# panuelosj/polystokes

Hardware: NVIDIA B200
Metric: stokes_steps_per_sec_256cubed (higher is better)
Workload: dtype f64

## Files before the change

### polystokes_b200/csrc/ps_api.cu

```cuda
#include "ps_solver.hpp"
#include <map>
#include <array>
#include <fstream>
#include <limits>
#include <thread>
#include <mutex>
#include <condition_variable>
#include <functional>
#include <memory>
#include <chrono>

using namespace ps;

struct MultiGroup;
struct ps_solver { Solver* S; void* tm[2] = {nullptr, nullptr}; Scratch scratch; MultiGroup* multi = nullptr; };

struct MultiGroup {
    struct Worker {
        std::thread th; std::mutex m; std::condition_variable cv;
        std::function<int()> task; bool has = false, quit = false, done = true; int rc = 0; std::string err;
        std::vector<void*> graveyard;
        const char* volatile where = "idle";
    };
    std::vector<ps_solver*> kids;
// ... 213 lines not shown
    if (name == "Mr") { out = blockdiag_csr(R ? S.RG.Mr.to_host(S.st, R * NN) : std::vector<double>(), R); return true; }
    if (name == "BInv") { out = blockdiag_csr(R ? S.RG.Binv.to_host(S.st, R * NN) : std::vector<double>(), R); return true; }
    if (name == "B") {
        std::vector<double> b(R * NN);
        if (R) { auto m = S.RG.Mr.to_host(S.st, R * NN); auto v = S.RG.Visc.to_host(S.st, R * NN); for (size_t i = 0; i < b.size(); ++i) b[i] = S.g.invDt * m[i] + 2. * v[i]; }
        out = blockdiag_csr(b, R); return true;
    }
    return false;
}
void mask_region_blocks(const Solver& S, const std::string& name, HostCsr& m) {
    if (!S.part.multi() || !(name == "Mr" || name == "B" || name == "BInv")) return;
    const size_t NN = (size_t)RDOF * RDOF;
    for (size_t i = 0; i < m.val.size(); ++i) { const int r = (int)(i / NN); if (r < S.RG.regLo || r >= S.RG.regHi) m.val[i] = 0.; }
}

bool get_vector(Solver& S, const std::string& n, std::vector<double>& out) {
    const Counts& C = S.C; const int R = S.RG.count; const size_t NN = (size_t)RDOF * RDOF;
    if (n == "activeRHS") out = S.rhsU.to_host(S.st, (size_t)C.nActiveVs);
    else if (n == "oldActiveVs") out = S.oldVs.to_host(S.st, (size_t)C.nActiveVs);
    else if (n == "reducedRHS") out = R ? S.RG.rhsR.to_host(S.st, (size_t)R * RDOF) : std::vector<double>();
    else if (n == "pressureRHS") out = S.rhsPT.to_host(S.st, (size_t)C.nPressures);
    else if (n == "stressRHS") { auto v = S.rhsPT.to_host(S.st, (size_t)C.nSystemSize); out.assign(v.begin() + C.nPressures, v.end()); }
    else if (n == "b") out = S.b.to_host(S.st, (size_t)C.nSystemSize);
    else if (n == "solution") out = S.x.to_host(S.st, (size_t)C.nSystemSize);
    else if (n == "velSolution") out = S.velSol.to_host(S.st, (size_t)(C.nActiveVs + C.nReducedVs));
    else if (n == "com") out = R ? S.RG.com.to_host(S.st, (size_t)3 * R) : std::vector<double>();
    else if (n == "bestFit") out = R ? S.RG.bestFit.to_host(S.st, (size_t)R * RDOF) : std::vector<double>();
    else if (n == "MrDense") out = R ? S.RG.Mr.to_host(S.st, R * NN) : std::vector<double>();
    else if (n == "ViscDense") out = R ? S.RG.Visc.to_host(S.st, R * NN) : std::vector<double>();
    else if (n == "BinvDense") out = R ? S.RG.Binv.to_host(S.st, R * NN) : std::vector<double>();
    else if (n == "guess") { if (S.guess.n < (size_t)C.nSystemSize) out.assign((size_t)C.nSystemSize, 0.); else out = S.guess.to_host(S.st, (size_t)C.nSystemSize); }
    else if (n == "diagA") { if (S.part.multi()) return false; S.computeDiagonal(); out = S.diagA.to_host(S.st, (size_t)C.nSystemSize); }
    else return false;
    if (S.part.multi()) {
        if (n == "b" || n == "solution") { for (size_t i = 0; i < out.size(); ++i) if (!S.ownSys.has((int64_t)i)) out[i] = 0.; }
        else if (n == "velSolution") {
            for (size_t i = 0; i < out.size(); ++i) {
                const bool mine = (int64_t)i < C.nActiveVs ? S.ownK.has((int64_t)i) : ((int64_t)(i - C.nActiveVs) / RDOF >= S.RG.regLo && (int64_t)(i - C.nActiveVs) / RDOF < S.RG.regHi);
                if (!mine) out[i] = 0.;
            }
        } else if (n == "reducedRHS" || n == "bestFit" || n == "MrDense" || n == "ViscDense" || n == "BinvDense") {
            const size_t per = (n == "reducedRHS" || n == "bestFit") ? (size_t)RDOF : NN;
            for (size_t i = 0; i < out.size(); ++i) { const int r = (int)(i / per); if (r < S.RG.regLo || r >= S.RG.regHi) out[i] = 0.; }
        }
    }
    return true;
}
// ... 199 lines not shown
    if (n == "nCenter") return C.nCenter;
    if (n == "nFaceX") return C.nFace[0]; if (n == "nFaceY") return C.nFace[1]; if (n == "nFaceZ") return C.nFace[2];
    if (n == "nEdgeYZ") return C.nEdge[0]; if (n == "nEdgeXZ") return C.nEdge[1]; if (n == "nEdgeXY") return C.nEdge[2];
    if (n == "nActiveVs") return C.nActiveVs; if (n == "nReducedVs") return C.nReducedVs;
    if (n == "nPressures") return C.nPressures; if (n == "nStresses") return C.nStresses;
    if (n == "nTotalDOFs") return C.nTotalDOFs; if (n == "nSystemSize") return C.nSystemSize;
    if (n == "regionCount") return S.RG.count; if (n == "iterations") return S.solveIterations;
    if (n == "peerTransport") return S.peer.on ? 1 : 0;
    if (n == "slabLocal") return S.part.local ? 1 : 0;
    if (n == "directHalo") return S.fusedHalo ? 1 : 0;
    if (n == "result") return S.result; if (n == "usedBiCGStab") return S.usedBiCGStab;
    if (n == "nRowsExt") return C.nRowsExt; if (n == "fixLoops") return S.fixLoops;
    if (n == "maxRegionRows") return S.RG.maxRegionRows; if (n == "maxRegionAxisRows") return S.RG.maxRegionAxisRows;
    if (n == "maxRegionCells") return S.RG.maxRegionCells; if (n == "minRegionCells") return S.RG.minRegionCells;
    if (n == "regionPath") return region_path(S.make_op_args(), S.RG);
    return INT64_MIN;
}
double ps_get_real(ps_handle h, const char* name) {
    if (!h || !name) return NAN;
    const std::string n(name);
    if (n == "solveError") return h->S->solveError;
    if (n == "xmag") return h->S->solveXmag;
    return NAN;
}

int64_t ps_get_index_field(ps_handle h, int kind, int slot, int32_t* out) {
    if (!h || slot < 0 || slot >= N_SLOTS || kind < 0 || kind > 2) return -1;
    if (h->multi) { g_lastError = "ps_get_index_field: per-voxel views of a ps_create_multi handle live on several GPUs; use a single-GPU handle"; return -1; }
    Solver& S = *h->S;
    const size_t n = (size_t)S.g.n[slot];
// ... 48 lines not shown
        dx.alloc(n); dy.alloc(n);
        copy_h2d(dx.p, x, n * sizeof(double), S.st);
        dy.zero(S.st, n);
        S.applyOperator(dx.p, dy.p, nullptr);
        copy_d2h(y, dy.p, n * sizeof(double), S.st);
        return (int)PS_SUCCESS;
    });
}

double ps_kernel_bytes(ps_handle h, const char* name) {
    if (!h || !name) return 0;
    const Solver& S = *h->S; const Counts& C = S.C; const std::string nm(name);
    const double nE = (double)(C.nEdge[0] + C.nEdge[1] + C.nEdge[2]);
    const double n = (double)C.nSystemSize;
    const double nRed = (double)S.RG.nRows;
    const double pass1Sweep = 32.0 * C.nRowsExt + 1.0 * C.nActiveVs  + 8.0 * n  + 8.0 * C.nRowsExt ;
    const double pass2 = 32.0 * C.nCenter + 20.0 * nE  + 8.0 * C.nRowsExt  + 8.0 * (C.nCenter + nE)
                       + 8.0 * n  + 8.0 * n ;
    const double pass2Dots = pass2 + 8.0 * n ;
    const double csrPass1 = 12.0 * 8.0 * C.nRowsExt + 8.0 * n + 8.0 * C.nActiveVs + 8.0 * C.nRowsExt;
    const double csrPass2 = 12.0 * (6.0 * C.nPressures + 2.0 * 3 * C.nCenter + 4.0 * nE) + 8.0 * C.nRowsExt + 8.0 * C.nStresses + 8.0 * C.nStresses + 8.0 * n;
    if (nm == "csr_pass1") return csrPass1;
    if (nm == "csr_pass2") return csrPass2;
    if (nm == "csr_apply") return csrPass1 + csrPass2 + nRed * 24.0 + (double)S.RG.count * (RDOF * RDOF + 2 * RDOF + 30) * 8.0;
    const double reduced = nRed * (8.0 + 4.0) + nRed * (4.0 + 8.0) + (double)S.RG.count * (RDOF * RDOF + 2 * RDOF + 30) * 8.0;
    const double pass1 = pass1Sweep + reduced;
    if (nm == "pass1") return pass1;
    if (nm == "pass1_sweep") return pass1Sweep;
    if (nm == "pass2") return pass2;
    if (nm == "pass2_dots") return pass2Dots;
    if (nm == "reduced") return reduced;
    if (nm == "apply") return pass1 + pass2;
// ... 112 lines not shown
```

### polystokes_b200/csrc/ps_assemble.cu

```cuda
#include "ps_solver.hpp"

namespace ps {

PS_D float local_viscosity_a(const Geom& g, const float* visc, int slot, const I3& idx) {
    int o[3] = {1, 1, 1};
    if (slot >= SL_FACE && slot < SL_EDGE) o[slot - SL_FACE] = 0;
    else if (slot >= SL_EDGE) { for (int a = 0; a < 3; ++a) if (a != slot - SL_EDGE) o[a] = 0; }
    const int b0 = o[0] ? idx.x : idx.x - 1, b1 = o[1] ? idx.y : idx.y - 1, b2 = o[2] ? idx.z : idx.z - 1;
    const float t0 = o[0] ? 0.f : 0.5f, t1 = o[1] ? 0.f : 0.5f, t2 = o[2] ? 0.f : 0.5f;
    float cz[2];
    for (int dz = 0; dz < 2; ++dz) {
        float cy[2];
        for (int dy = 0; dy < 2; ++dy) {
            const float a = float_at(g, visc, SL_CENTER, I3{b0, b1 + dy, b2 + dz});
            const float b = float_at(g, visc, SL_CENTER, I3{b0 + 1, b1 + dy, b2 + dz});
            cy[dy] = fadd_rn(a, fmul_rn(t0, fsub_rn(b, a)));
        }
        cz[dz] = fadd_rn(cy[0], fmul_rn(t1, fsub_rn(cy[1], cy[0])));
    }
    return fadd_rn(cz[0], fmul_rn(t2, fsub_rn(cz[1], cz[0])));
}

PS_D double clampd(double v, double lo, double hi) { return fmin(fmax(v, lo), hi); }

// ... 178 lines not shown
                }
            }
            const int64_t erow = eRowOff + ei;
            ecode[erow] = (uint32_t)word;
            for (int k = 0; k < 4; ++k) ecol[(int64_t)k * nERows + erow] = cidx[k];
            rhsPT[nP + tOff + ei] = rhs;
            const double volumeWeight = clampd((double)fwe * 0.125, MINWEIGHT, 1.0) * ((double)lw * 0.125);
            const double localViscosity = (double)local_viscosity_a(g, visc, SL_EDGE + e, ed);
            const double invLocalViscosity = clampd(1. / localViscosity, 0., 1e10);
            uInv[tOff + ei] = mul_rn(mul_rn(2., invLocalViscosity), volumeWeight);
            uDiag[tOff + ei] = mul_rn(mul_rn(0.5, localViscosity), clampd(1. / volumeWeight, 0., 1.e2));
        });
    }
}

}
```

### polystokes_b200/csrc/ps_pcg.cu

```cuda
#include "ps_solver.hpp"
#include "ps_peer.hpp"

namespace ps {

PS_D double k_row(const OpArgs& A, int64_t r, const double* __restrict__ x) {
    const uint64_t word = A.kcode[r];
    const int32_t c0w = A.kcol[r];
    const int64_t cOff = A.nP + (int64_t)((uint32_t)c0w >> 30) * A.nC;
    int64_t col[8];
    col[0] = c0w & OP_COL_MASK; col[1] = A.kcol[A.nRowsExt + r]; col[2] = cOff + col[0]; col[3] = cOff + col[1];
    for (int k = 0; k < 4; ++k) col[4 + k] = A.kcol[(int64_t)(2 + k) * A.nRowsExt + r];
    double s = 0.;
    for (int k = 0; k < 8; ++k) { const int code = op_code(word, k); if (code) s += ((double)code * A.valScale) * x[col[k]]; }
    return s;
}
PS_D void kt_cell_rows(const OpArgs& A, int64_t ci, const double* __restrict__ w, double* out) {
    const uint64_t word = A.ccode[ci];
    double v[6], wv[6];
    for (int k = 0; k < 6; ++k) { const int code = op_code(word, k); v[k] = (double)code * A.valScale; wv[k] = code ? w[A.ccol[(int64_t)k * A.nC + ci]] : 0.; }
    double s = 0.;
    for (int k = 0; k < 6; ++k) s += v[k] * wv[k];
    out[0] = s;
    for (int a = 0; a < 3; ++a) { double t = 0.; t += (-v[2 * a]) * wv[2 * a]; t += (-v[2 * a + 1]) * wv[2 * a + 1]; out[1 + a] = t; }
}
PS_D double kt_edge_row(const OpArgs& A, int64_t e, const double* __restrict__ w) {
    const uint64_t word = A.ecode[e];
    double s = 0.;
    for (int k = 0; k < 4; ++k) { const int code = op_code(word, k); if (code) s += ((double)code * A.valScale) * w[A.ecol[(int64_t)k * A.nE + e]]; }
    return s;
}

PS_D void moments_to_t(const double* M, double* t) {
    for (int n = 0; n < RDOF; ++n) t[n] = 0.;
    const double* A = M; const double* B = M + 10; const double* Cz = M + 20;
    t[0] = A[0]; t[3] = A[1]; t[4] = A[2]; t[5] = A[3]; for (int k = 0; k < 6; ++k) t[6 + k] = A[4 + k];
    t[1] = B[0]; t[12] = B[1]; t[13] = B[2]; t[14] = B[3]; for (int k = 0; k < 6; ++k) t[15 + k] = B[4 + k];
    t[2] += Cz[0]; t[3] += -Cz[3]; t[6] += -2. * Cz[6]; t[7] += -Cz[8]; t[8] += -0.5 * Cz[9];
    t[13] += -Cz[3]; t[16] += -Cz[6]; t[18] += -2. * Cz[8]; t[19] += -0.5 * Cz[9];
    t[21] += Cz[1]; t[22] += Cz[2]; t[23] += Cz[4]; t[24] += Cz[5]; t[25] += Cz[7];
}
PS_D void s_to_sigma(const double* s, double* sg) {
    sg[0] = s[0]; sg[1] = s[3]; sg[2] = s[4]; sg[3] = s[5]; for (int k = 0; k < 6; ++k) sg[4 + k] = s[6 + k];
    sg[10] = s[1]; sg[11] = s[12]; sg[12] = s[13]; sg[13] = s[14]; for (int k = 0; k < 6; ++k) sg[14 + k] = s[15 + k];
// ... 57 lines not shown
    for (int i = threadIdx.x; i < n; i += HOT_THREADS) s += __ldcg(p + i);
    return block_sum(s);
}
__device__ __forceinline__ bool last_block(unsigned int* ticket) {
    __shared__ bool last;
    if (threadIdx.x == 0) {
        __threadfence();
        const unsigned t = atomicInc(ticket, gridDim.x - 1);
        last = (t == gridDim.x - 1);
        if (last) __threadfence();
    }
    __syncthreads();
    return last;
}

__device__ __forceinline__ void pass1_block(const OpArgs& A, const double* __restrict__ x, double* __restrict__ w, double activeScale, const double* lut, int32_t e) {
    const int k = (int)((uint32_t)e >> 28);
    const int64_t r = A.s1.lo[k] + (int64_t)(e & 0x0fffffff) * SCHED_BLOCK + threadIdx.x;
    if (r >= A.s1.hi[k]) return;
    const double sc = A.valScale;
    const uint64_t word = __ldcs(A.kcode + r);
    int32_t c[6];
#pragma unroll
    for (int k2 = 0; k2 < 6; ++k2) c[k2] = __ldcs(A.kcol + (int64_t)k2 * A.nRowsExt + r);
    const int64_t cOff = A.nP + (int64_t)((uint32_t)c[0] >> 30) * A.nC;
    const int64_t c0 = c[0] & OP_COL_MASK, c1 = c[1];
    const int64_t col[8] = {c0, c1, cOff + c0, cOff + c1, c[2], c[3], c[4], c[5]};
    double xv[8];
#pragma unroll
    for (int k2 = 0; k2 < 8; ++k2) xv[k2] = ((word >> (8 * k2)) & 0xffull) ? x[col[k2]] : 0.;
    double s = 0.;
#pragma unroll
    for (int k2 = 0; k2 < 8; ++k2) s += ((double)op_code(word, k2) * sc) * xv[k2];
    w[r] = r < A.nActiveVs ? activeScale * lut[__ldcs(A.kmc + r)] * s : s;
}
__global__ void __launch_bounds__(HOT_THREADS, 6) pass1_kernel(const __grid_constant__ OpArgs A, const double* __restrict__ x, double* __restrict__ w, double activeScale, const PcgScalars* S, int reverse,
                                                             const int32_t* __restrict__ sched, int nSched, const __grid_constant__ VecLink V) {    pdl_sync();

    __shared__ double lut[65];
// ... 15 lines not shown
__global__ void __launch_bounds__(HOT_THREADS, OCC) pass2_kernel(const __grid_constant__ OpArgs A, const double* __restrict__ w, const double* __restrict__ x, double* __restrict__ y,
                                                              double muScale, const double* __restrict__ add, double* dotPartial, PcgScalars* S, int mode, const __grid_constant__ PeerCtx P,
                                                              const double* __restrict__ r2, int reverse, const __grid_constant__ VecLink V) {    pdl_sync();

    if (S && S->done) return;
    if (blockIdx.x == 0 && threadIdx.x == 0) vec_raise(V);
    if (!vec_wait(V)) { if (threadIdx.x == 0) S->peerError = 1; return; }
    const bool dot = mode & 1, dot3 = mode & 2;
    const double sc = A.valScale;
    const int64_t nC = A.nC, nP = A.nP, oE = A.nP + 3 * A.nC;
    double acc = 0., accR = 0., accY = 0.;
#pragma unroll 1
    for (int g = blockIdx.x; g < A.nSched2; g += gridDim.x) {
        const int32_t se = __ldg(A.sched2 + (reverse ? A.nSched2 - 1 - g : g));
        const int k = (int)((uint32_t)se >> 28);
        const int64_t row = A.s2.lo[k] + (int64_t)(se & 0x0fffffff) * SCHED_BLOCK + threadIdx.x;
        if (row >= A.s2.hi[k]) continue;
        if (k == 0) {
            const int64_t ci = row;
            const uint64_t word = __ldcs(A.ccode + ci);
            double v[6], wv[6];
#pragma unroll
            for (int q = 0; q < 6; ++q) {
                const int32_t c = __ldcs(A.ccol + (int64_t)q * nC + ci);
                v[q] = (double)op_code(word, q) * sc;
                wv[q] = ((word >> (8 * q)) & 0xffull) ? w[c] : 0.;
            }
            double s = 0.;
#pragma unroll
            for (int q = 0; q < 6; ++q) s += v[q] * wv[q];
            double yp = -s;
            if (add) yp += add[ci];
            y[ci] = yp;
            if (dot) acc += x[ci] * yp;
            if (dot3) { accR += r2[ci] * yp; accY += yp * yp; }
            const double ui = muScale != 0. ? muScale * A.uInv[ci] : 0.;
#pragma unroll
            for (int a = 0; a < 3; ++a) {
                double t = 0.;
                t += (-v[2 * a]) * wv[2 * a]; t += (-v[2 * a + 1]) * wv[2 * a + 1];
                const int64_t jj = nP + a * nC + ci;
                const double xj = x ? x[jj] : 0.;
                double yt = -t;
                if (muScale != 0.) yt -= ui * xj;
                if (add) yt += add[jj];
                y[jj] = yt;
                acc += xj * yt;
                if (dot3) { accR += r2[jj] * yt; accY += yt * yt; }
            }
        } else {
            const int64_t e = row;
            const uint32_t word = __ldcs(A.ecode + e);
            double s = 0.;
#pragma unroll
            for (int q = 0; q < 4; ++q) {
                const int32_t c = __ldcs(A.ecol + (int64_t)q * A.nE + e);
                const double wv = ((word >> (8 * q)) & 0xffu) ? w[c] : 0.;
                s += ((double)op_code(word, q) * sc) * wv;
            }
            const int64_t jj = oE + e;
            const double xj = x ? x[jj] : 0.;
            double yt = -s;
            if (muScale != 0.) yt -= muScale * A.uInv[3 * nC + e] * xj;
            if (add) yt += add[jj];
            y[jj] = yt;
            acc += xj * yt;
            if (dot3) { accR += r2[jj] * yt; accY += yt * yt; }
        }
    }
    if (dot) {
        const double bs = block_sum(acc);
        if (threadIdx.x == 0) dotPartial[blockIdx.x] = bs;
// ... 1055 lines not shown
```

### polystokes_b200/csrc/ps_solver.cu

```cuda
#include "ps_solver.hpp"
#include <climits>
#include <chrono>
#include <memory>
#include <unistd.h>

namespace ps {

thread_local std::string g_lastError;
thread_local int64_t g_launches = 0;
thread_local Scratch* g_scratch = nullptr;
thread_local std::vector<void*>* g_deferredFree = nullptr;
thread_local const char* volatile* g_where = nullptr;

static void k_flag_label(cudaStream_t st, int64_t lo, int64_t hi, const int8_t* L, int value, uint8_t* flag) {
    ps_for_range(st, lo, hi, PS_LAMBDA(int64_t q) { flag[q] = (L[q] == value) ? 1 : 0; });
}
static void k_krow_active(cudaStream_t st, int64_t lo, int64_t hi, const int32_t* aidx, int32_t offset, int32_t* krow) {
    ps_for_range(st, lo, hi, PS_LAMBDA(int64_t q) { const int a = aidx[q]; krow[q] = a >= 0 ? a + offset : -1; });
}
static void k_krow_reduced(cudaStream_t st, int64_t nRows, const int32_t* rowFace, int32_t base, int32_t* kr0, int32_t* kr1, int32_t* kr2) {
    ps_for(st, nRows, PS_LAMBDA(int64_t i) {
        const int32_t packed = rowFace[i];
        const int axis = (packed >> 29) & 3;
        int32_t* kr = axis == 0 ? kr0 : axis == 1 ? kr1 : kr2;
// ... 706 lines not shown
    C.nRowsExt = C.nActiveVs + RG.nRows;
    const int64_t nE = C.nEdge[0] + C.nEdge[1] + C.nEdge[2];
    Op.alloc(C.nRowsExt, C.nActiveVs, C.nCenter, nE);
    mcInv.alloc((size_t)C.nActiveVs); mc.alloc((size_t)C.nActiveVs); rhsU.alloc((size_t)C.nActiveVs); oldVs.alloc((size_t)C.nActiveVs);
    computeOwnership();
    RowSet allRows; allRows.add(0, C.nRowsExt);
    k_assemble_K(st, g, F, C, Op, mcInv.p, mc.p, rhsU.p, oldVs.p, part.local ? ownK : allRows);
    uInv.alloc((size_t)C.nStresses); uDiag.alloc((size_t)C.nStresses); rhsPT.alloc((size_t)C.nSystemSize);
    k_assemble_Kt(st, g, F, C, Op, uInv.p, uDiag.p, rhsPT.p, part.local);
    const size_t n = (size_t)C.nSystemSize;
    b.alloc(n); x.alloc(n); r.alloc(n); Ap.alloc(n); allocVectors(n, (size_t)C.nRowsExt + 1);
    velSol.alloc((size_t)(C.nActiveVs + C.nReducedVs) + 1);
    dotPartial.alloc(3 * 16384);
    computeOwnership();
    buildSchedules();
    buildHalos();
    exchangeVectorPointers();
}

void Solver::allocVectors(size_t n, size_t nRows) {
#ifndef PS_EMULATE
    if (peer.on) {
        const size_t offW = (n + 31) & ~(size_t)31;
        const size_t need = offW + nRows;
        if (!vecArena.p || vecArena.n < need) {
            if (arenaGraveyard) { dev_free(arenaGraveyard); arenaGraveyard = nullptr; }
            arenaGraveyard = vecArena.release();
            vecArena.alloc(std::max(need + need / 8, (size_t)1 << 19));
        }
        p.adopt(vecArena.p, n); w.adopt(vecArena.p + offW, nRows);
// ... 211 lines not shown
    if (kind == 0) k_halo_push_p(st, H.nSend[0], H.nSend[1], H.sendIdx.p, r.p, p.p, Ap.p, dst[0], dst[1], scal.p, *updateCtx);
    else k_halo_push_direct(st, H.nSend[0], H.nSend[1], H.sendIdx.p, w.p, dst[0], dst[1], scal.p);
#else
    (void)H; (void)kind; (void)updateCtx;
#endif
    return L;
}
void Solver::allreduce(double* devBuf, int n) { if (part.multi() && comm && !peer.on) comm->allreduce_sum(devBuf, n, st); }

static OpArgs make_op(const Solver& S) {
    OpArgs A;
    A.nRowsExt = S.C.nRowsExt; A.nActiveVs = S.C.nActiveVs; A.nP = S.C.nPressures; A.nT = S.C.nStresses; A.nC = S.C.nCenter;
    A.nE = S.C.nEdge[0] + S.C.nEdge[1] + S.C.nEdge[2];
    A.kcode = S.Op.kcode.p; A.kcol = S.Op.kcol.p; A.kmc = S.Op.kmc.p; A.mcInvLut = S.Op.mcInvLut.p;
    A.ccode = S.Op.ccode.p; A.ccol = S.Op.ccol.p; A.ecode = S.Op.ecode.p; A.ecol = S.Op.ecol.p;
    A.uInv = S.uInv.p; A.valScale = S.g.invDx / 64.;
    A.rowsK = S.ownK; A.rowsP = S.ownP; A.rowsE = S.ownE;
    A.s1 = S.sr1; A.s2 = S.sr2; A.sched1 = S.sched1.p; A.sched2 = S.sched2.p; A.nSched1 = S.nSched1; A.nSched2 = S.nSched2;
    A.sched1a = S.sched1a.p; A.sched1b = S.sched1b.p; A.nSched1a = S.nSched1a; A.nSched1b = S.nSched1b;
    return A;
}
OpArgs Solver::make_op_args() const { return make_op(*this); }

void Solver::pass1Apply(const OpArgs& A, const double* xin, const PcgScalars* S, bool reverse, const VecLink& V) {
#ifndef PS_EMULATE
    if (RG.count > 0 && !reverse && k_pass1_regions(st, A, xin, w.p, g.dt, S, g, RG, 1.0, V)) return;
#endif
    k_pass1(st, A, xin, w.p, g.dt, S, reverse, 0, V);
    if (RG.count > 0) reduced_apply(st, g, RG, w.p + C.nActiveVs, 1.0, S);
}
// ... 420 lines not shown
```

### polystokes_b200/csrc/ps_solver.hpp

```cpp
#pragma once
#include "ps_grid.hpp"
#include "ps_part.hpp"
#include "ps_comm.hpp"
#include "ps_peer.hpp"
#include "../../include/polystokes_b200.h"

namespace ps {

struct CompactOp {
    int64_t nRows = 0, nCells = 0, nEdges = 0;
    DBuf<uint64_t> kcode;
    DBuf<int32_t> kcol;
    DBuf<uint8_t> kmc;
    DBuf<double> mcInvLut;
    DBuf<uint64_t> ccode;
    DBuf<int32_t> ccol;
    DBuf<uint32_t> ecode;
    DBuf<int32_t> ecol;
    void alloc(int64_t rows, int64_t nAct, int64_t cells, int64_t edges) {
        nRows = rows; nCells = cells; nEdges = edges;
        kcode.alloc((size_t)rows + 1); kcol.alloc((size_t)6 * rows + 1); kmc.alloc((size_t)nAct + 1); mcInvLut.alloc(65);
        ccode.alloc((size_t)cells + 1); ccol.alloc((size_t)6 * cells + 1); ecode.alloc((size_t)edges + 1); ecol.alloc((size_t)4 * edges + 1);
    }
};
PS_HD int op_code(uint64_t word, int k) { return (int)(int8_t)(uint8_t)(word >> (8 * k)); }
constexpr int32_t OP_COL_MASK = 0x3fffffff;

constexpr int SCHED_BLOCK = 256;
struct SchedRanges {
    int n = 0;
    int64_t lo[4] = {0, 0, 0, 0}, hi[4] = {0, 0, 0, 0};
    int64_t items[4] = {-1, -1, -1, -1};
    void add(int64_t a, int64_t b) { lo[n] = a; hi[n] = b > a ? b : a; ++n; }
    void addItems(int64_t first, int64_t count) { lo[n] = first; hi[n] = first + (count > 0 ? count : 0); items[n] = count > 0 ? count : 0; ++n; }
    int64_t blocks(int k) const { return items[k] >= 0 ? items[k] : (hi[k] - lo[k] + SCHED_BLOCK - 1) / SCHED_BLOCK; }
};
std::vector<int32_t> merge_schedule(const SchedRanges& R);

struct RegionData {
    int32_t count = 0;
    DBuf<double> com;
    DBuf<double> Mr, Visc, N, Binv;
    DBuf<double> lsqRhs, bestFit, rhsR;
    DBuf<double> moments;
    DBuf<double> tables;
    DBuf<int32_t> cellList;
    DBuf<int32_t> cellStart;
    int64_t nRows = 0;
    DBuf<int32_t> rowFace;
    DBuf<uint32_t> rowXYZ;
// ... 206 lines not shown
void k_valid_faces(cudaStream_t, const Geom&, const Fields&, float* const valid[3]);

int64_t tile_order_scan(cudaStream_t, const Geom&, int slot, const uint8_t* flag, int32_t* out, DBuf<int32_t>& tileCounts,
                        const std::vector<int>* zCut = nullptr, std::vector<int64_t>* cuts = nullptr, const int* tileZ = nullptr);
int64_t exclusive_scan_i64(cudaStream_t, int64_t n, const int64_t* in, int64_t* out);
void sort_pairs_by_key(cudaStream_t, int64_t n, int keyBits, DBuf<int32_t>& keys, DBuf<int32_t>& vals, DBuf<int32_t>& keysTmp, DBuf<int32_t>& valsTmp);

void k_region_com(cudaStream_t, const Geom&, const Fields&, int32_t R, unsigned long long* sums, double* com);
void k_collect_region_keys(cudaStream_t, const Geom&, const int32_t* rank, const uint8_t* flag, const int32_t* region, int64_t lo, int64_t hi, int32_t tag, int32_t rankOffset, int32_t* keys, int32_t* vals);
void region_gram_partials(cudaStream_t, const Geom&, const Fields&, const RegionData&, double* partial);
void region_gram_finish(cudaStream_t, const Geom&, RegionData&, int nChunks);
void k_flag_coupled_faces(cudaStream_t, const Geom&, const Fields&, int axis, uint8_t* flag, int32_t regLo, int32_t regHi, int64_t lo, int64_t hi);

void k_assemble_K(cudaStream_t, const Geom&, const Fields&, const Counts&, CompactOp& Op, double* mcInv, double* mc, double* rhsU, double* oldVs, const RowSet& ownRows);
void k_assemble_Kt(cudaStream_t, const Geom&, const Fields&, const Counts&, CompactOp& Op, double* uInv, double* uDiag, double* rhsPT, bool ownOnly);

struct OpArgs {
    int64_t nRowsExt, nActiveVs, nP, nT, nC, nE;
    SchedRanges s1, s2;
    const int32_t* sched1; const int32_t* sched2; int nSched1, nSched2;
    const int32_t* sched1a; const int32_t* sched1b; int nSched1a, nSched1b;
    RowSet rowsK, rowsP, rowsE;
    const uint64_t* kcode; const int32_t* kcol; const uint8_t* kmc; const double* mcInvLut;
    const uint64_t* ccode; const int32_t* ccol; const uint32_t* ecode; const int32_t* ecol;
    const double* uInv;
    double valScale;
};
void k_pass1(cudaStream_t, const OpArgs&, const double* x, double* w, double activeScale, const PcgScalars* scal, bool reverse = false, int part = 0, const VecLink& V = VecLink());
#ifndef PS_EMULATE
bool k_pass1_regions(cudaStream_t, const OpArgs&, const double* x, double* w, double activeScale, const PcgScalars* scal, const Geom&, const RegionData&, double scale, const VecLink& V = VecLink());
#endif
void k_pass2(cudaStream_t, const OpArgs&, const double* w, const double* x, double* y, double muScale, const double* add, double* dotPartial, const PeerCtx& P, PcgScalars* scal, int mode,
             const double* r2 = nullptr, bool reverse = false, const VecLink& V = VecLink());
void reduced_moments(cudaStream_t, const Geom&, const RegionData&, const double* wRows, const PcgScalars* scal, bool solve = false);
void reduced_finish(cudaStream_t, const Geom&, const RegionData&, const double* extraRhs, double extraScale, double tScale, const PcgScalars* scal);
void reduced_expand(cudaStream_t, const Geom&, const RegionData&, double* wRows, double scale, const PcgScalars* scal);
void reduced_apply(cudaStream_t, const Geom&, const RegionData&, double* wRows, double scale, const PcgScalars* scal);
int region_path(const OpArgs&, const RegionData&);
void k_cg_update(cudaStream_t, const RangeSet& own, double* x, double* r, double* p, const double* Ap, double* dotPartial, PcgScalars* scal, const PeerCtx& P, bool reverse = false, const VecLink& V = VecLink());
void k_cg_init(cudaStream_t, const RangeSet& own, const double* b, double* x, double* r, double* p, double* dotPartial, PcgScalars* scal, double tol, int maxIter, const PeerCtx& P);
void k_cg_begin(cudaStream_t, PcgScalars* scal, const PeerCtx& P);
void k_bicg_init(cudaStream_t, const RangeSet& own, const double* b, double* x, double* r, double* rhat, double* p, double* v, PcgScalars* scal, double tol, int maxIter);
// ... 41 lines not shown
```

Baseline: 7.641.

## Compress operator column indices to 16-bit per-block offsets with headers

Adds a setup pass that encodes each schedule block's int32 column indices as 16-bit offsets against per-block base values stored in a 64-byte header, falling back to the full-width arrays for blocks whose range is too wide. The pass1 and pass2 operator kernels now read the uint16 offsets and reconstruct columns, roughly halving index traffic in these bandwidth-bound sweeps. This costs extra header loads, a few integer ops per entry, extra device memory and setup work. It also adds debug accessors and updates the bandwidth model to account for the packed sizes.

```diff
diff --git a/polystokes_b200/csrc/ps_api.cu b/polystokes_b200/csrc/ps_api.cu
--- a/polystokes_b200/csrc/ps_api.cu
+++ b/polystokes_b200/csrc/ps_api.cu
@@ -251,6 +251,45 @@
     for (size_t i = 0; i < m.val.size(); ++i) { const int r = (int)(i / NN); if (r < S.RG.regLo || r >= S.RG.regHi) m.val[i] = 0.; }
 }
 
+std::vector<double> op_columns(Solver& S, int pass, bool packed) {
+    OpArgs A = S.make_op_args();
+    const int64_t nR = S.C.nRowsExt, nC = S.C.nCenter, nE = A.nE;
+    std::vector<uint64_t> kcode, ccode; std::vector<uint32_t> ecode; std::vector<int32_t> kcol, ccol, ecol, h1, h2; std::vector<uint16_t> koff, coff, eoff;
+    std::vector<double> out;
+    if (pass == 1) {
+        kcode = S.Op.kcode.to_host(S.st, (size_t)nR); kcol = S.Op.kcol.to_host(S.st, (size_t)6 * nR); koff = S.Op.koff.to_host(S.st, (size_t)6 * nR);
+        h1 = S.Op.hdr1.to_host(S.st, (size_t)S.sr1.totalBlocks() * PACK_HDR);
+        A.kcode = kcode.data(); A.kcol = kcol.data(); A.koff = koff.data(); A.hdr1 = h1.data();
+        out.assign((size_t)6 * nR, -1.);
+        for (int64_t r = 0; r < nR; ++r) {
+            if (A.s1.rangeOf(r) < 0) continue;
+            const uint64_t word = kcode[(size_t)r];
+            for (int s = 0; s < 6; ++s) {
+                const uint32_t c = (uint32_t)(packed ? op_col1(A, r, s) : kcol[(size_t)(s * nR + r)]);
+                if (kcol_used(word, s)) out[(size_t)(s * nR + r)] = (double)c;
+                else if (s == 0 && kcol_used(word, 1)) out[(size_t)r] = (double)(c & ~(uint32_t)OP_COL_MASK);
+            }
+        }
+        return out;
+    }
+    ccode = S.Op.ccode.to_host(S.st, (size_t)nC); ccol = S.Op.ccol.to_host(S.st, (size_t)6 * nC); coff = S.Op.coff.to_host(S.st, (size_t)6 * nC);
+    ecode = S.Op.ecode.to_host(S.st, (size_t)nE); ecol = S.Op.ecol.to_host(S.st, (size_t)4 * nE); eoff = S.Op.eoff.to_host(S.st, (size_t)4 * nE);
+    h2 = S.Op.hdr2.to_host(S.st, (size_t)S.sr2.totalBlocks() * PACK_HDR);
+    A.ccode = ccode.data(); A.ccol = ccol.data(); A.coff = coff.data(); A.ecode = ecode.data(); A.ecol = ecol.data(); A.eoff = eoff.data(); A.hdr2 = h2.data();
+    out.assign((size_t)(6 * nC + 4 * nE), -1.);
+    for (int k = 0; k < A.s2.n; ++k)
+        for (int64_t r = A.s2.lo[k]; r < A.s2.hi[k]; ++r) {
+            const bool cell = k == 0;
+            const uint64_t word = cell ? ccode[(size_t)r] : (uint64_t)ecode[(size_t)r];
+            for (int s = 0; s < (cell ? 6 : 4); ++s) {
+                if (!((word >> (8 * s)) & 0xffull)) continue;
+                const size_t i = cell ? (size_t)(s * nC + r) : (size_t)(6 * nC + s * nE + r);
+                out[i] = (double)(packed ? op_col2(A, cell, r, s) : (cell ? ccol : ecol)[(size_t)(s * (cell ? nC : nE) + r)]);
+            }
+        }
+    return out;
+}
+
 bool get_vector(Solver& S, const std::string& n, std::vector<double>& out) {
     const Counts& C = S.C; const int R = S.RG.count; const size_t NN = (size_t)RDOF * RDOF;
     if (n == "activeRHS") out = S.rhsU.to_host(S.st, (size_t)C.nActiveVs);
@@ -268,6 +307,8 @@
     else if (n == "BinvDense") out = R ? S.RG.Binv.to_host(S.st, R * NN) : std::vector<double>();
     else if (n == "guess") { if (S.guess.n < (size_t)C.nSystemSize) out.assign((size_t)C.nSystemSize, 0.); else out = S.guess.to_host(S.st, (size_t)C.nSystemSize); }
     else if (n == "diagA") { if (S.part.multi()) return false; S.computeDiagonal(); out = S.diagA.to_host(S.st, (size_t)C.nSystemSize); }
+    else if (n == "opColumns1" || n == "opColumns1Packed") out = op_columns(S, 1, n != "opColumns1");
+    else if (n == "opColumns2" || n == "opColumns2Packed") out = op_columns(S, 2, n != "opColumns2");
     else return false;
     if (S.part.multi()) {
         if (n == "b" || n == "solution") { for (size_t i = 0; i < out.size(); ++i) if (!S.ownSys.has((int64_t)i)) out[i] = 0.; }
@@ -497,6 +538,8 @@
     if (n == "maxRegionRows") return S.RG.maxRegionRows; if (n == "maxRegionAxisRows") return S.RG.maxRegionAxisRows;
     if (n == "maxRegionCells") return S.RG.maxRegionCells; if (n == "minRegionCells") return S.RG.minRegionCells;
     if (n == "regionPath") return region_path(S.make_op_args(), S.RG);
+    if (n == "packedBlocks1") return pack_counts(S.st, S.Op, S.sr1, 1).packedBlocks; if (n == "wideBlocks1") return pack_counts(S.st, S.Op, S.sr1, 1).wideBlocks;
+    if (n == "packedBlocks2") return pack_counts(S.st, S.Op, S.sr2, 2).packedBlocks; if (n == "wideBlocks2") return pack_counts(S.st, S.Op, S.sr2, 2).wideBlocks;
     return INT64_MIN;
 }
 double ps_get_real(ps_handle h, const char* name) {
@@ -575,8 +618,12 @@
     const double nE = (double)(C.nEdge[0] + C.nEdge[1] + C.nEdge[2]);
     const double n = (double)C.nSystemSize;
     const double nRed = (double)S.RG.nRows;
-    const double pass1Sweep = 32.0 * C.nRowsExt + 1.0 * C.nActiveVs  + 8.0 * n  + 8.0 * C.nRowsExt ;
-    const double pass2 = 32.0 * C.nCenter + 20.0 * nE  + 8.0 * C.nRowsExt  + 8.0 * (C.nCenter + nE)
+    auto columns = [&](const SchedRanges& R, int pass) {
+        const PackCounts k = pack_counts(S.st, S.Op, R, pass);
+        return 2.0 * k.packedEntries + 4.0 * k.wideEntries + (double)PACK_HDR * 4 * (k.packedBlocks + k.wideBlocks);
+    };
+    const double pass1Sweep = 8.0 * C.nRowsExt + columns(S.sr1, 1) + 1.0 * C.nActiveVs  + 8.0 * n  + 8.0 * C.nRowsExt ;
+    const double pass2 = 8.0 * C.nCenter + 4.0 * nE + columns(S.sr2, 2)  + 8.0 * C.nRowsExt  + 8.0 * (C.nCenter + nE)
                        + 8.0 * n  + 8.0 * n ;
     const double pass2Dots = pass2 + 8.0 * n ;
     const double csrPass1 = 12.0 * 8.0 * C.nRowsExt + 8.0 * n + 8.0 * C.nActiveVs + 8.0 * C.nRowsExt;
diff --git a/polystokes_b200/csrc/ps_assemble.cu b/polystokes_b200/csrc/ps_assemble.cu
--- a/polystokes_b200/csrc/ps_assemble.cu
+++ b/polystokes_b200/csrc/ps_assemble.cu
@@ -216,4 +216,121 @@
     }
 }
 
-}
+PS_HD uint16_t pack_off(int32_t c, int32_t lb, int32_t hb) {
+    const uint32_t d = (uint32_t)c - (uint32_t)lb;
+    return (uint16_t)(d <= 0x7fffu ? d : (uint32_t)c - (uint32_t)hb);
+}
+#ifndef PS_EMULATE
+__device__ __forceinline__ int32_t warp_min_i(int32_t v) { return __reduce_min_sync(0xffffffffu, v); }
+__device__ __forceinline__ int32_t warp_max_i(int32_t v) { return __reduce_max_sync(0xffffffffu, v); }
+__device__ __forceinline__ bool warp_leader() { return (threadIdx.x & 31) == 0; }
+#else
+inline int32_t warp_min_i(int32_t v) { return v; }
+inline int32_t warp_max_i(int32_t v) { return v; }
+inline bool warp_leader() { return true; }
+#endif
+struct KCols {
+    const uint64_t* code; const int32_t* col; uint16_t* off; int64_t n;
+    PS_HD int slots(int) const { return 6; }
+    PS_HD int32_t get(int, int64_t r, int s) const { return kcol_used(code[r], s) ? (col[s * n + r] & OP_COL_MASK) : -1; }
+    PS_HD int axis(int, int64_t r) const { return (code[r] & 0xffffffffull) ? (int)((uint32_t)col[r] >> 30) : -1; }
+    PS_HD uint16_t* dst(int, int s) const { return off + s * n; }
+};
+struct KtCols {
+    const uint64_t* ccode; const int32_t* ccol; uint16_t* coff; int64_t nC;
+    const uint32_t* ecode; const int32_t* ecol; uint16_t* eoff; int64_t nE;
+    PS_HD int slots(int k) const { return k == 0 ? 6 : 4; }
+    PS_HD int32_t get(int k, int64_t r, int s) const {
+        if (k == 0) return ((ccode[r] >> (8 * s)) & 0xffull) ? ccol[s * nC + r] : -1;
+        return ((ecode[r] >> (8 * s)) & 0xffu) ? ecol[s * nE + r] : -1;
+    }
+    PS_HD int axis(int, int64_t) const { return -1; }
+    PS_HD uint16_t* dst(int k, int s) const { return k == 0 ? coff + s * nC : eoff + s * nE; }
+};
+constexpr int PACK_TMP = 24;
+template <class Acc>
+static void encode_sweep(cudaStream_t st, const SchedRanges& sr, const Acc a, int32_t* hdr, int32_t* T) {
+    const SchedRanges R = sr;
+    const int64_t nb = R.totalBlocks();
+    if (nb <= 0) return;
+    ps_for(st, nb * PACK_TMP, PS_LAMBDA(int64_t i) { const int j = (int)(i % PACK_TMP); T[i] = (j >= 6 && j < 12) || j == 13 ? -1 : INT32_MAX; });
+    ps_for(st, nb * SCHED_BLOCK, PS_LAMBDA(int64_t t) {
+        const int64_t b = t / SCHED_BLOCK;
+        int64_t lo, hi; const int k = R.blockRows(b, lo, hi);
+        const int64_t r = lo + (t - b * SCHED_BLOCK); const bool in = r < hi;
+        int32_t* Tb = T + b * PACK_TMP;
+        for (int s = 0; s < a.slots(k); ++s) {
+            const int32_t c = in ? a.get(k, r, s) : -1;
+            const int32_t mn = warp_min_i(c >= 0 ? c : INT32_MAX), mx = warp_max_i(c);
+            if (warp_leader() && mx >= 0) { atomic_min(Tb + s, mn); atomic_max(Tb + 6 + s, mx); }
+        }
+        const int ax = in ? a.axis(k, r) : -1;
+        const int32_t amn = warp_min_i(ax >= 0 ? ax : INT32_MAX), amx = warp_max_i(ax);
+        if (warp_leader() && amx >= 0) { atomic_min(Tb + 12, amn); atomic_max(Tb + 13, amx); }
+    });
+    ps_for(st, nb * SCHED_BLOCK, PS_LAMBDA(int64_t t) {
+        const int64_t b = t / SCHED_BLOCK;
+        int64_t lo, hi; const int k = R.blockRows(b, lo, hi);
+        const int64_t r = lo + (t - b * SCHED_BLOCK); const bool in = r < hi;
+        int32_t* Tb = T + b * PACK_TMP;
+        for (int s = 0; s < a.slots(k); ++s) {
+            const int32_t mn = Tb[s], mx = Tb[6 + s];
+            if (mx < 0 || mx - mn <= 0xffff) continue;
+            const int32_t c = in ? a.get(k, r, s) : -1;
+            const int32_t m2 = warp_min_i(c > mn + 0x7fff ? c : INT32_MAX);
+            if (warp_leader() && m2 != INT32_MAX) atomic_min(Tb + 16 + s, m2);
+        }
+    });
+    ps_for(st, nb, PS_LAMBDA(int64_t b) {
+        const int32_t* Tb = T + b * PACK_TMP;
+        int32_t* h = hdr + b * PACK_HDR;
+        int wide = 0;
+        const bool anyAxis = Tb[13] >= 0;
+        if (anyAxis && Tb[12] != Tb[13]) wide |= 1;
+        const int32_t ax = (int32_t)((uint32_t)(anyAxis ? Tb[13] : 0) << 30);
+        for (int s = 0; s < 6; ++s) {
+            const int32_t mn = Tb[s], mx = Tb[6 + s];
+            int32_t lb = 0, hb = 0;
+            if (mx >= 0 && mx - mn <= 0xffff) lb = hb = mn;
+            else if (mx >= 0) { lb = mn; hb = Tb[16 + s] - 0x8000; if (mx - Tb[16 + s] > 0x7fff) wide |= 1 << s; }
+            if (s == 0) { lb |= ax; hb |= ax; }
+            h[2 * s] = lb; h[2 * s + 1] = hb;
+        }
+        h[PACK_WIDE] = wide; h[13] = h[14] = h[15] = 0;
+    });
+    ps_for(st, nb * SCHED_BLOCK, PS_LAMBDA(int64_t t) {
+        const int64_t b = t / SCHED_BLOCK;
+        const int32_t* h = hdr + b * PACK_HDR;
+        if (h[PACK_WIDE]) return;
+        int64_t lo, hi; const int k = R.blockRows(b, lo, hi);
+        const int64_t r = lo + (t - b * SCHED_BLOCK);
+        if (r >= hi) return;
+        for (int s = 0; s < a.slots(k); ++s) {
+            const int32_t c = a.get(k, r, s);
+            a.dst(k, s)[r] = c >= 0 ? pack_off(c, h[2 * s] & OP_COL_MASK, h[2 * s + 1] & OP_COL_MASK) : (uint16_t)0;
+        }
+    });
+}
+void pack_columns(cudaStream_t st, const Counts& C, CompactOp& Op, const SchedRanges& s1, const SchedRanges& s2) {
+    const int64_t nb1 = s1.totalBlocks(), nb2 = s2.totalBlocks();
+    Op.hdr1.alloc((size_t)nb1 * PACK_HDR + 1); Op.hdr2.alloc((size_t)nb2 * PACK_HDR + 1);
+    Op.packTmp.alloc((size_t)std::max(nb1, nb2) * PACK_TMP + 1);
+    const int64_t nE = C.nEdge[0] + C.nEdge[1] + C.nEdge[2];
+    encode_sweep(st, s1, KCols{Op.kcode.p, Op.kcol.p, Op.koff.p, C.nRowsExt}, Op.hdr1.p, Op.packTmp.p);
+    encode_sweep(st, s2, KtCols{Op.ccode.p, Op.ccol.p, Op.coff.p, C.nCenter, Op.ecode.p, Op.ecol.p, Op.eoff.p, nE}, Op.hdr2.p, Op.packTmp.p);
+}
+PackCounts pack_counts(cudaStream_t st, const CompactOp& Op, const SchedRanges& R, int pass) {
+    PackCounts c;
+    const int64_t nb = R.totalBlocks();
+    if (nb <= 0) return c;
+    const std::vector<int32_t> h = (pass == 1 ? Op.hdr1 : Op.hdr2).to_host(st, (size_t)nb * PACK_HDR);
+    for (int64_t b = 0; b < nb; ++b) {
+        int64_t lo, hi;
+        const int k = R.blockRows(b, lo, hi);
+        const int64_t entries = (hi - lo) * (pass == 2 && k > 0 ? 4 : 6);
+        if (h[(size_t)b * PACK_HDR + PACK_WIDE]) { ++c.wideBlocks; c.wideEntries += entries; } else { ++c.packedBlocks; c.packedEntries += entries; }
+    }
+    return c;
+}
+
+}
diff --git a/polystokes_b200/csrc/ps_pcg.cu b/polystokes_b200/csrc/ps_pcg.cu
--- a/polystokes_b200/csrc/ps_pcg.cu
+++ b/polystokes_b200/csrc/ps_pcg.cu
@@ -5,11 +5,11 @@
 
 PS_D double k_row(const OpArgs& A, int64_t r, const double* __restrict__ x) {
     const uint64_t word = A.kcode[r];
-    const int32_t c0w = A.kcol[r];
+    const int32_t c0w = op_col1(A, r, 0);
     const int64_t cOff = A.nP + (int64_t)((uint32_t)c0w >> 30) * A.nC;
     int64_t col[8];
-    col[0] = c0w & OP_COL_MASK; col[1] = A.kcol[A.nRowsExt + r]; col[2] = cOff + col[0]; col[3] = cOff + col[1];
-    for (int k = 0; k < 4; ++k) col[4 + k] = A.kcol[(int64_t)(2 + k) * A.nRowsExt + r];
+    col[0] = c0w & OP_COL_MASK; col[1] = op_col1(A, r, 1); col[2] = cOff + col[0]; col[3] = cOff + col[1];
+    for (int k = 0; k < 4; ++k) col[4 + k] = op_col1(A, r, 2 + k);
     double s = 0.;
     for (int k = 0; k < 8; ++k) { const int code = op_code(word, k); if (code) s += ((double)code * A.valScale) * x[col[k]]; }
     return s;
@@ -17,7 +17,7 @@
 PS_D void kt_cell_rows(const OpArgs& A, int64_t ci, const double* __restrict__ w, double* out) {
     const uint64_t word = A.ccode[ci];
     double v[6], wv[6];
-    for (int k = 0; k < 6; ++k) { const int code = op_code(word, k); v[k] = (double)code * A.valScale; wv[k] = code ? w[A.ccol[(int64_t)k * A.nC + ci]] : 0.; }
+    for (int k = 0; k < 6; ++k) { const int code = op_code(word, k); v[k] = (double)code * A.valScale; wv[k] = code ? w[op_col2(A, true, ci, k)] : 0.; }
     double s = 0.;
     for (int k = 0; k < 6; ++k) s += v[k] * wv[k];
     out[0] = s;
@@ -26,7 +26,7 @@
 PS_D double kt_edge_row(const OpArgs& A, int64_t e, const double* __restrict__ w) {
     const uint64_t word = A.ecode[e];
     double s = 0.;
-    for (int k = 0; k < 4; ++k) { const int code = op_code(word, k); if (code) s += ((double)code * A.valScale) * w[A.ecol[(int64_t)k * A.nE + e]]; }
+    for (int k = 0; k < 4; ++k) { const int code = op_code(word, k); if (code) s += ((double)code * A.valScale) * w[op_col2(A, false, e, k)]; }
     return s;
 }
 
@@ -114,15 +114,32 @@
     return last;
 }
 
+template <int NS>
+__device__ __forceinline__ void block_columns(const int32_t* h, const uint16_t* __restrict__ off, const int32_t* __restrict__ wide, int64_t stride, int64_t r, int32_t* c) {
+    const int4* h4 = reinterpret_cast<const int4*>(h);
+    const int4 b0 = __ldg(h4), b1 = __ldg(h4 + 1), b2 = __ldg(h4 + 2), b3 = __ldg(h4 + 3);
+    uint32_t o[NS];
+#pragma unroll
+    for (int q = 0; q < NS; ++q) o[q] = __ldcs(off + (int64_t)q * stride + r);
+    const int32_t lo[6] = {b0.x, b0.z, b1.x, b1.z, b2.x, b2.z}, hi[6] = {b0.y, b0.w, b1.y, b1.w, b2.y, b2.w};
+#pragma unroll
+    for (int q = 0; q < NS; ++q) c[q] = pack_col(o[q], lo[q], hi[q]);
+    static_assert(PACK_WIDE == 12, "the wide mask is the first word of the header's last 16 bytes");
+    if (b3.x) {
+#pragma unroll
+        for (int q = 0; q < NS; ++q) c[q] = __ldcs(wide + (int64_t)q * stride + r);
+    }
+}
+
 __device__ __forceinline__ void pass1_block(const OpArgs& A, const double* __restrict__ x, double* __restrict__ w, double activeScale, const double* lut, int32_t e) {
     const int k = (int)((uint32_t)e >> 28);
-    const int64_t r = A.s1.lo[k] + (int64_t)(e & 0x0fffffff) * SCHED_BLOCK + threadIdx.x;
+    const int64_t j = e & 0x0fffffff;
+    const int64_t r = A.s1.lo[k] + j * SCHED_BLOCK + threadIdx.x;
     if (r >= A.s1.hi[k]) return;
     const double sc = A.valScale;
     const uint64_t word = __ldcs(A.kcode + r);
     int32_t c[6];
-#pragma unroll
-    for (int k2 = 0; k2 < 6; ++k2) c[k2] = __ldcs(A.kcol + (int64_t)k2 * A.nRowsExt + r);
+    block_columns<6>(A.hdr1 + (A.s1.first[k] + j) * PACK_HDR, A.koff, A.kcol, A.nRowsExt, r, c);
     const int64_t cOff = A.nP + (int64_t)((uint32_t)c[0] >> 30) * A.nC;
     const int64_t c0 = c[0] & OP_COL_MASK, c1 = c[1];
     const int64_t col[8] = {c0, c1, cOff + c0, cOff + c1, c[2], c[3], c[4], c[5]};
@@ -168,17 +185,20 @@
     for (int g = blockIdx.x; g < A.nSched2; g += gridDim.x) {
         const int32_t se = __ldg(A.sched2 + (reverse ? A.nSched2 - 1 - g : g));
         const int k = (int)((uint32_t)se >> 28);
-        const int64_t row = A.s2.lo[k] + (int64_t)(se & 0x0fffffff) * SCHED_BLOCK + threadIdx.x;
+        const int64_t j = se & 0x0fffffff;
+        const int64_t row = A.s2.lo[k] + j * SCHED_BLOCK + threadIdx.x;
         if (row >= A.s2.hi[k]) continue;
+        const int32_t* h = A.hdr2 + (A.s2.first[k] + j) * PACK_HDR;
         if (k == 0) {
             const int64_t ci = row;
             const uint64_t word = __ldcs(A.ccode + ci);
+            int32_t c[6];
+            block_columns<6>(h, A.coff, A.ccol, nC, ci, c);
             double v[6], wv[6];
 #pragma unroll
             for (int q = 0; q < 6; ++q) {
-                const int32_t c = __ldcs(A.ccol + (int64_t)q * nC + ci);
                 v[q] = (double)op_code(word, q) * sc;
-                wv[q] = ((word >> (8 * q)) & 0xffull) ? w[c] : 0.;
+                wv[q] = ((word >> (8 * q)) & 0xffull) ? w[c[q]] : 0.;
             }
             double s = 0.;
 #pragma unroll
@@ -205,11 +225,12 @@
         } else {
             const int64_t e = row;
             const uint32_t word = __ldcs(A.ecode + e);
+            int32_t c[4];
+            block_columns<4>(h, A.eoff, A.ecol, A.nE, e, c);
             double s = 0.;
 #pragma unroll
             for (int q = 0; q < 4; ++q) {
-                const int32_t c = __ldcs(A.ecol + (int64_t)q * A.nE + e);
-                const double wv = ((word >> (8 * q)) & 0xffu) ? w[c] : 0.;
+                const double wv = ((word >> (8 * q)) & 0xffu) ? w[c[q]] : 0.;
                 s += ((double)op_code(word, q) * sc) * wv;
             }
             const int64_t jj = oE + e;
diff --git a/polystokes_b200/csrc/ps_solver.cu b/polystokes_b200/csrc/ps_solver.cu
--- a/polystokes_b200/csrc/ps_solver.cu
+++ b/polystokes_b200/csrc/ps_solver.cu
@@ -744,6 +744,7 @@
     dotPartial.alloc(3 * 16384);
     computeOwnership();
     buildSchedules();
+    pack_columns(st, C, Op, sr1, sr2);
     buildHalos();
     exchangeVectorPointers();
 }
@@ -985,6 +986,7 @@
     A.nE = S.C.nEdge[0] + S.C.nEdge[1] + S.C.nEdge[2];
     A.kcode = S.Op.kcode.p; A.kcol = S.Op.kcol.p; A.kmc = S.Op.kmc.p; A.mcInvLut = S.Op.mcInvLut.p;
     A.ccode = S.Op.ccode.p; A.ccol = S.Op.ccol.p; A.ecode = S.Op.ecode.p; A.ecol = S.Op.ecol.p;
+    A.koff = S.Op.koff.p; A.coff = S.Op.coff.p; A.eoff = S.Op.eoff.p; A.hdr1 = S.Op.hdr1.p; A.hdr2 = S.Op.hdr2.p;
     A.uInv = S.uInv.p; A.valScale = S.g.invDx / 64.;
     A.rowsK = S.ownK; A.rowsP = S.ownP; A.rowsE = S.ownE;
     A.s1 = S.sr1; A.s2 = S.sr2; A.sched1 = S.sched1.p; A.sched2 = S.sched2.p; A.nSched1 = S.nSched1; A.nSched2 = S.nSched2;
diff --git a/polystokes_b200/csrc/ps_solver.hpp b/polystokes_b200/csrc/ps_solver.hpp
--- a/polystokes_b200/csrc/ps_solver.hpp
+++ b/polystokes_b200/csrc/ps_solver.hpp
@@ -17,23 +17,41 @@
     DBuf<int32_t> ccol;
     DBuf<uint32_t> ecode;
     DBuf<int32_t> ecol;
+    DBuf<uint16_t> koff, coff, eoff;
+    DBuf<int32_t> hdr1, hdr2;
+    DBuf<int32_t> packTmp;
     void alloc(int64_t rows, int64_t nAct, int64_t cells, int64_t edges) {
         nRows = rows; nCells = cells; nEdges = edges;
         kcode.alloc((size_t)rows + 1); kcol.alloc((size_t)6 * rows + 1); kmc.alloc((size_t)nAct + 1); mcInvLut.alloc(65);
         ccode.alloc((size_t)cells + 1); ccol.alloc((size_t)6 * cells + 1); ecode.alloc((size_t)edges + 1); ecol.alloc((size_t)4 * edges + 1);
+        koff.alloc((size_t)6 * rows + 1); coff.alloc((size_t)6 * cells + 1); eoff.alloc((size_t)4 * edges + 1);
     }
 };
 PS_HD int op_code(uint64_t word, int k) { return (int)(int8_t)(uint8_t)(word >> (8 * k)); }
 constexpr int32_t OP_COL_MASK = 0x3fffffff;
+PS_HD bool kcol_used(uint64_t word, int s) { return s < 2 ? ((word >> (8 * s)) & 0xff00ffull) != 0 : ((word >> (8 * (s + 2))) & 0xffull) != 0; }
+
+constexpr int PACK_HDR = 16, PACK_WIDE = 12;
+PS_HD int32_t pack_col(uint32_t off, int32_t lo, int32_t hi) { return (int32_t)(off + (uint32_t)(off < 0x8000u ? lo : hi)); }
 
 constexpr int SCHED_BLOCK = 256;
 struct SchedRanges {
     int n = 0;
     int64_t lo[4] = {0, 0, 0, 0}, hi[4] = {0, 0, 0, 0};
     int64_t items[4] = {-1, -1, -1, -1};
-    void add(int64_t a, int64_t b) { lo[n] = a; hi[n] = b > a ? b : a; ++n; }
-    void addItems(int64_t first, int64_t count) { lo[n] = first; hi[n] = first + (count > 0 ? count : 0); items[n] = count > 0 ? count : 0; ++n; }
+    int64_t first[5] = {0, 0, 0, 0, 0};
+    void add(int64_t a, int64_t b) { lo[n] = a; hi[n] = b > a ? b : a; ++n; first[n] = first[n - 1] + blocks(n - 1); }
+    void addItems(int64_t first_, int64_t count) { lo[n] = first_; hi[n] = first_ + (count > 0 ? count : 0); items[n] = count > 0 ? count : 0; ++n; first[n] = first[n - 1] + blocks(n - 1); }
     int64_t blocks(int k) const { return items[k] >= 0 ? items[k] : (hi[k] - lo[k] + SCHED_BLOCK - 1) / SCHED_BLOCK; }
+    int64_t totalBlocks() const { return first[n]; }
+    PS_HD int rangeOf(int64_t r) const { for (int k = 0; k < n; ++k) if (r >= lo[k] && r < hi[k]) return k; return -1; }
+    PS_HD int64_t blockOf(int k, int64_t r) const { return first[k] + (r - lo[k]) / SCHED_BLOCK; }
+    PS_HD int blockRows(int64_t b, int64_t& rlo, int64_t& rhi) const {
+        int k = 0;
+        while (k + 1 < n && b >= first[k + 1]) ++k;
+        rlo = lo[k] + (b - first[k]) * SCHED_BLOCK; rhi = rlo + SCHED_BLOCK < hi[k] ? rlo + SCHED_BLOCK : hi[k];
+        return k;
+    }
 };
 std::vector<int32_t> merge_schedule(const SchedRanges& R);
 
@@ -270,6 +288,9 @@
 
 void k_assemble_K(cudaStream_t, const Geom&, const Fields&, const Counts&, CompactOp& Op, double* mcInv, double* mc, double* rhsU, double* oldVs, const RowSet& ownRows);
 void k_assemble_Kt(cudaStream_t, const Geom&, const Fields&, const Counts&, CompactOp& Op, double* uInv, double* uDiag, double* rhsPT, bool ownOnly);
+void pack_columns(cudaStream_t, const Counts&, CompactOp& Op, const SchedRanges& s1, const SchedRanges& s2);
+struct PackCounts { int64_t packedBlocks = 0, wideBlocks = 0, packedEntries = 0, wideEntries = 0; };
+PackCounts pack_counts(cudaStream_t, const CompactOp& Op, const SchedRanges& R, int pass);
 
 struct OpArgs {
     int64_t nRowsExt, nActiveVs, nP, nT, nC, nE;
@@ -279,9 +300,27 @@
     RowSet rowsK, rowsP, rowsE;
     const uint64_t* kcode; const int32_t* kcol; const uint8_t* kmc; const double* mcInvLut;
     const uint64_t* ccode; const int32_t* ccol; const uint32_t* ecode; const int32_t* ecol;
+    const uint16_t* koff; const uint16_t* coff; const uint16_t* eoff; const int32_t* hdr1; const int32_t* hdr2;
     const double* uInv;
     double valScale;
 };
+PS_HD int32_t op_col1(const OpArgs& A, int64_t r, int s) {
+    const int k = A.s1.rangeOf(r);
+    const int64_t i = (int64_t)s * A.nRowsExt + r;
+    if (k < 0) return A.kcol[i];
+    const int32_t* h = A.hdr1 + A.s1.blockOf(k, r) * PACK_HDR;
+    return h[PACK_WIDE] ? A.kcol[i] : pack_col(A.koff[i], h[2 * s], h[2 * s + 1]);
+}
+PS_HD int32_t op_col2(const OpArgs& A, bool cell, int64_t r, int s) {
+    int k = -1;
+    if (cell) { if (A.s2.n > 0 && r >= A.s2.lo[0] && r < A.s2.hi[0]) k = 0; }
+    else for (int j = 1; j < A.s2.n; ++j) if (r >= A.s2.lo[j] && r < A.s2.hi[j]) k = j;
+    const int64_t i = (int64_t)s * (cell ? A.nC : A.nE) + r;
+    const int32_t* wide = cell ? A.ccol : A.ecol;
+    if (k < 0) return wide[i];
+    const int32_t* h = A.hdr2 + A.s2.blockOf(k, r) * PACK_HDR;
+    return h[PACK_WIDE] ? wide[i] : pack_col((cell ? A.coff : A.eoff)[i], h[2 * s], h[2 * s + 1]);
+}
 void k_pass1(cudaStream_t, const OpArgs&, const double* x, double* w, double activeScale, const PcgScalars* scal, bool reverse = false, int part = 0, const VecLink& V = VecLink());
 #ifndef PS_EMULATE
 bool k_pass1_regions(cudaStream_t, const OpArgs&, const double* x, double* w, double activeScale, const PcgScalars* scal, const Geom&, const RegionData&, double scale, const VecLink& V = VecLink());
```

Result: slower. 7.304, median of 6 (-4.4%).
